# michael-fonder/M4Depth

Measured on AMD Instinct MI355X. Metric: frames/s, higher is better.
Workload: dtype f32

## Files before the change

include/m4depth_hip.h:

```cpp
#ifndef M4DEPTH_HIP_H_
#define M4DEPTH_HIP_H_

#include <stdint.h>

#ifdef __cplusplus
extern "C" {
#endif

#define M4D_ABI_VERSION 6

int m4d_abi_version(void);
long long m4d_launch_count(void);
const char* m4d_build_info(void);
const char* m4d_switches_info(void);


int m4d_backproject_fwd(const float* input, const float* coords, const int dims[6],
                        float* out, void* stream);

int m4d_backproject_bwd(const float* grad, const float* input, const float* coords,
                        const int dims[6], float* input_grad, float* coords_grad, void* stream);


int m4d_dense_image_warp(const float* image, const float* flow, int B, int H, int W, int C,
// ... 7 lines not shown
                       const float* cam_f, const float* cam_c, int b, int h, int w,
                       float* out, void* stream);
int m4d_depth2parallax(const float* depth, const float* rot, int rot_c, const float* trans,
                       const float* cam_f, const float* cam_c, int b, int h, int w,
                       float* out, void* stream);
int m4d_prev_d2para(const float* prev_d, const float* rot, int rot_c, const float* trans,
                    const float* cam_f, const float* cam_c, int b, int h, int w,
                    float* out, void* stream);
int m4d_reproject_flow(const float* depth, const float* rot, int rot_c, const float* trans,
                       const float* cam_f, const float* cam_c, int b, int h, int w,
                       float* flow, float* proj_minus_rot, float* rot_coord, void* stream);
int m4d_recompute_depth(const float* depth, const float* rot, int rot_c, const float* trans,
                        const float* cam_f, const float* cam_c, int b, int h, int w,
                        float* out, void* stream);


int m4d_dscv_fwd(const float* c1, const float* c2, const float* disp_prev_t, const float* disp,
                 const float* rot, int rot_c, const float* trans, const float* cam_f,
                 const float* cam_c, int b, int h, int w, int C, int search_range, int nbre_cuts,
                 int cv_accum, float* cv, int cv_stride, float* prev_disp,
                 float* log_center, int log_stride, float log_scale,
                 int32_t* index_out, void* stream);

void m4d_dscv_set_variant(int variant);
void m4d_dscv_set_fallback_counter(unsigned int* device_counter);
void m4d_dscv_set_ablation(int mask);
void m4d_dscv_set_stamps(unsigned long long* device_buffer);

int m4d_sncv_fwd(const float* c1, const float* c2, int b, int h, int w, int C, int search_range,
                 int dilation_rate, int nbre_cuts, float* out, int out_stride, void* stream);
int m4d_dscv_sncv_fwd(const float* c1, const float* c2, const float* disp_prev_t, const float* disp,
                      const float* rot, int rot_c, const float* trans, const float* cam_f,
                      const float* cam_c, int b, int h, int w, int C, int search_range, int nbre_cuts,
                      int cv_accum, float* cv, int cv_stride, float* prev_disp,
                      float* log_center, int log_stride, float log_scale,
                      int sncv_search_range, float* sncv_out, int sncv_out_stride, void* stream);

int m4d_conv3x3_wino_bias_act(const float* x, const float* wu, const float* bias, int b, int h, int w,
                              int Cin, int Cout, int CoutPad, float slope, float* out, void* stream);
int m4d_conv3x3_wino2_bias_act(const float* x, const float* wu8, const float* bias, int b, int h, int w,
                               int Cin, int Cout, int CoutPad, float slope, float* out, void* stream);
void m4d_wino_set_stamps(unsigned long long* device_buffer);
int m4d_conv3x3_wino6_bias_act(const float* x, const void* wu6, const float* bias, int b, int h, int w,
                               int Cin, int Cout, int CoutPad, float slope, float* out, void* stream);
int m4d_conv3x3_wino6_bias_act_k(const float* x, const void* wu6, const float* bias, int b, int h, int w,
                                 int Cin, int Cout, int CoutPad, float slope, float* out, int kernel, void* stream);
long long m4d_wino6_persistent_min_units(void);
void m4d_wino6_set_stamps(unsigned long long* device_buffer);
int m4d_conv3x3_wino6_bias_act_ks(const float* x, const void* wu6, const float* bias, int b, int h, int w,
                                  int Cin, int Cout, int CoutPad, float slope, float* out, int kernel,
                                  int stagger_us, int stagger_phases, void* stream);
int m4d_conv3x3_winof16_bias_act_ks(const float* x, const void* wuh, const float* bias, int b, int h, int w,
                                    int Cin, int Cout, int CoutPad, float slope, float* out,
                                    int stagger_us, int stagger_phases, void* stream);

int m4d_refiner_tail(const float* x32, const float* w6p, const float* b6, const float* w7p, const float* b7,
                     const float* rot, int rot_c, const float* trans, const float* cam_f, const float* cam_c,
                     int b, int h, int w, float scale, float* parallax, float* depth, float* other,
                     float* depth_state, void* stream);
int m4d_refiner_tail6(const float* x32, const void* w6f, const float* b6, const void* w7f, const float* b7,
                      const float* rot, int rot_c, const float* trans, const float* cam_f, const float* cam_c,
                      int b, int h, int w, float scale, float* parallax, float* depth, float* other,
                      float* depth_state, void* stream);

int m4d_refiner_tail6_m(const float* x32, const void* w6f, const float* b6, const void* w7f, const float* b7,
                        const float* rot, int rot_c, const float* trans, const float* cam_f, const float* cam_c,
                        int b, int h, int w, float scale, float* parallax, float* depth, float* other,
                        float* depth_state, const unsigned char* reset, float reset_parallax, void* stream);
int m4d_refiner_tail_m(const float* x32, const float* w6p, const float* b6, const float* w7p, const float* b7,
                       const float* rot, int rot_c, const float* trans, const float* cam_f, const float* cam_c,
                       int b, int h, int w, float scale, float* parallax, float* depth, float* other,
                       float* depth_state, const unsigned char* reset, float reset_parallax, void* stream);
int m4d_level_post_m(const float* refiner_out, const float* rot, int rot_c, const float* trans,
                     const float* cam_f, const float* cam_c, int b, int h, int w, float scale,
                     float* parallax, float* depth, float* other, float* depth_state,
                     const unsigned char* reset, float reset_parallax, void* stream);
int m4d_stream_prepare(const unsigned char* new_traj, int force_all, const float* rot, int rot_c, const float* trans,
                       int b, unsigned char* reset, float* rot_out, float* trans_out, void* stream);


int m4d_dscv_bwd(const float* c1, const float* c2, const float* disp_prev_t, const float* disp,
                 const float* rot, int rot_c, const float* trans, const float* cam_f,
                 const float* cam_c, int b, int h, int w, int C, int search_range, int nbre_cuts,
                 const float* g_cv, int g_cv_stride, const float* g_prev_disp,
                 float* g_c1, float* g_c2, float* g_disp, float* g_disp_prev_t, void* stream);

int m4d_sncv_bwd(const float* c1, const float* c2, const float* out, int out_stride,
                 const float* g, int g_stride, int b, int h, int w, int C, int search_range,
                 int dilation_rate, int nbre_cuts, float slope, float* g_c1, float* g_c2,
                 void* stream);


int m4d_resize_bilinear_v1_bwd(const float* g_out, int b, int ih, int iw, int c, int oh, int ow,
                               float mul, float* g_in, void* stream);
int m4d_level_post_bwd(const float* refiner_out, const float* g_parallax, const float* g_depth,
                       const float* g_other, const float* rot, int rot_c, const float* trans,
                       const float* cam_f, const float* cam_c, int b, int h, int w, float scale,
                       float* g_refiner_out, void* stream);
int m4d_normalize_cuts_bwd(const float* x, const float* g, int b, int h, int w, int C, int nbre_cuts,
                           float* g_x, void* stream);
long long m4d_bias_act_bwd_workspace_floats(long long rows, int C);
int m4d_bias_act_bwd(const float* g, const float* out, long long rows, int C, float slope,
                     float* g_pre, float* g_bias, float* workspace, void* stream);
int m4d_pack_conv_weights(const float* w_ohwi, int O, int I, int transpose, float* wp, void* stream);
int m4d_pack_conv_weights_lat(const float* w_ohwi, int O, int I, int transpose, void* wp, void* stream);
long long m4d_loss_workspace_floats(void);
// ... 235 lines not shown
```

m4depth_amd/csrc/m4d_wino_f16.hip:

```cpp
#include <cstdlib>
#include "m4d_common.h"
#include "../../include/m4depth_hip.h"

namespace {

typedef float f32x16 __attribute__((ext_vector_type(16)));
typedef _Float16 f16x8 __attribute__((ext_vector_type(8)));
typedef unsigned u32x4 __attribute__((ext_vector_type(4)));
typedef int i32x4 __attribute__((ext_vector_type(4)));

struct WinoF16Args {
  const float* x; const unsigned char* wu; const short* wexp; const float* bias; float* out;
  int b, h, w, Cin, Cout, CoutPad, n_chunks, tiles_x, tiles_y;
  float slope;
  int phases;
  int stagger;
};

constexpr int kT = 16, kH = kT + 2;
constexpr int kJ = 10;
constexpr int kPix = 5;
constexpr int kRow = 2 * kJ * kPix;
constexpr int kRawUsed = kH * kRow;
constexpr int kRawDma = 29;
constexpr int kRawK = 4;
constexpr int kRawSlots = kRawDma * 64;
constexpr int kFrag = 4 * 1024;
constexpr int kBRingBytes = 4 * kFrag;
constexpr int kBRingOff = 2 * kRawSlots * 16;
constexpr int kEpiBytes = (4 * 4 * 2 * 32 * 36 + 32) * 4;
constexpr int kPmOff = kEpiBytes;
constexpr int kTsOff = kPmOff + kH * kH * 4;
constexpr int kLdsBytes = kTsOff + 16 * 64 * 4;
static_assert(kBRingOff + 4 * kBRingBytes <= kEpiBytes, "the K loop's LDS lies inside the epilogue's");
static_assert(kLdsBytes <= 160 * 1024, "LDS budget of one CU");

__device__ __forceinline__ void split2_pair(float v0, float v1, float S, unsigned& hi, unsigned& lo) {
  asm("v_fma_mixlo_f16 %0, %1, %2, 0" : "=v"(hi) : "v"(v0), "v"(S));
  asm("v_fma_mixhi_f16 %0, %1, %2, 0" : "+v"(hi) : "v"(v1), "v"(S));
  asm("v_fma_mixlo_f16 %0, %1, %2, -%3 op_sel_hi:[0,0,1]" : "=v"(lo) : "v"(v0), "v"(S), "v"(hi));
  asm("v_fma_mixhi_f16 %0, %1, %2, -%3 op_sel:[0,0,1] op_sel_hi:[0,0,1]" : "+v"(lo) : "v"(v1), "v"(S), "v"(hi));
}

__device__ __forceinline__ float max3_abs(float m, float a, float b) {
  asm("v_max3_f32 %0, %0, |%1|, |%2|" : "+v"(m) : "v"(a), "v"(b));
  return m;
}

__global__ void __launch_bounds__(512) __attribute__((amdgpu_waves_per_eu(2, 2)))
conv3x3_winof16_kernel(const WinoF16Args a) {
  extern __shared__ __align__(16) float lds[];
  asm volatile("" : : "s"(a.x), "s"(a.wu), "s"(a.out), "s"(a.bias));
  if (a.stagger > 0 && blockIdx.y == 0 && blockIdx.x < 256) {
    const unsigned phase = (blockIdx.x >> 3) & (unsigned)(a.phases - 1);
    const unsigned long long t_end = wall_clock64() + (unsigned long long)(phase * (unsigned)a.stagger) / (unsigned)a.phases;
    for (int spin = 0; spin < 512 && wall_clock64() < t_end; ++spin) __builtin_amdgcn_s_sleep(16);
  }
  float4* raw = reinterpret_cast<float4*>(lds);
  unsigned* pm = reinterpret_cast<unsigned*>(reinterpret_cast<unsigned char*>(lds) + kPmOff);
  int* ts = reinterpret_cast<int*>(reinterpret_cast<unsigned char*>(lds) + kTsOff);
  const unsigned lds_base = (unsigned)(size_t)(__attribute__((address_space(3))) float*)lds;

  const int t = threadIdx.x, lane = t & 63;
  const int wv = __builtin_amdgcn_readfirstlane(t >> 6);
  const int pr = wv & 3, mt = wv >> 2;
// ... 59 lines not shown
        const int c = c0 + 2 * cc;
        const int s = src0 + qq + ((c & 1) * kJ + (c >> 1)) * kPix;
        const float4 da = rbuf[s + ra * kRow], db = rbuf[s + rb_ * kRow];
        tv[c][4 * qq + 0] = __builtin_fmaf(sgn, db.x, da.x);
        tv[c][4 * qq + 1] = __builtin_fmaf(sgn, db.y, da.y);
        tv[c][4 * qq + 2] = __builtin_fmaf(sgn, db.z, da.z);
        tv[c][4 * qq + 3] = __builtin_fmaf(sgn, db.w, da.w);
      }
  };
  float Sc[4];
  auto gen_pair = [&](int c, int e, u32x4 (&A)[2]) {
    float v[2];
#pragma unroll
    for (int h = 0; h < 2; ++h) {
      const int ch = 2 * e + h;
      v[h] = c == 0 ? tv[0][ch] - tv[2][ch] : c == 1 ? tv[1][ch] + tv[2][ch] : c == 2 ? tv[2][ch] - tv[1][ch] : tv[1][ch] - tv[3][ch];
    }
    unsigned p_hi, p_lo;
    split2_pair(v[0], v[1], Sc[c], p_hi, p_lo);
    A[0][e] = p_hi; A[1][e] = p_lo;
  };

  const long long w_pos = kFrag;
  const long long w_chunk = (long long)n_groups * 16 * w_pos;
  const unsigned char* wc = a.wu + ((long long)ng * 16 + 4 * pr) * w_pos;
  const unsigned bring = lds_base + (unsigned)(kBRingOff + pr * kBRingBytes);
  const unsigned char* bring_p = reinterpret_cast<const unsigned char*>(lds) + kBRingOff + pr * kBRingBytes;
  const unsigned bl = (unsigned)lane * 16u;
  const bool half = __builtin_amdgcn_readfirstlane(ng * 64 + 32 >= a.Cout ? 1 : 0) != 0;
  const unsigned bl_dma = (half && mt == 1) ? 0u : bl + (unsigned)mt * 2048u;
  auto b_dma = [&](const unsigned char* gsrc, int slot) {
    asm volatile("s_mov_b32 m0, %1\n\ts_nop 0\n\t"
                 "global_load_lds_dwordx4 %0, %2\n\tglobal_load_lds_dwordx4 %0, %2 offset:1024"
                 : : "v"(bl_dma), "s"(bring + (unsigned)(slot * kFrag) + (unsigned)mt * 2048u), "s"(gsrc) : "memory", "m0");
  };
  f16x8 B0[2][2], B1[2];
  auto frag = [&](int slot, int nt, int part) {
    return *reinterpret_cast<const f16x8*>(bring_p + slot * kFrag + (nt * 2 + part) * 1024 + bl);
  };
#define M4D_WF_WAIT(nn) asm volatile("s_waitcnt vmcnt(" #nn ") lgkmcnt(0)" ::: "memory")

  f32x16 acc[4][2];

#pragma unroll
  for (int k = 0; k < kRawK; ++k) raw_dma(0, 0, k);
  b_dma(wc, 0);
  b_dma(wc + w_pos, 1);
  b_dma(wc + 2 * w_pos, 2);
#pragma unroll
  for (int k = 0; k < kRawK; ++k) raw_dma(min(1, last), 1, k);
  b_dma(wc + 3 * w_pos, 3);
  static_assert(kRawK == 4, "the vmcnt counts below assume 4 raw-halo pieces + 2 fragment pieces per position");

  {
    const int g = t & 7, p0 = t >> 3, nq = a.Cin >> 2;
    constexpr int kR = (kH * kH + 63) / 64;
    int poff[kR];
    bool pv[kR];
    float mx[kR];
#pragma unroll
    for (int r = 0; r < kR; ++r) {
      const int p = p0 + 64 * r, hy = p / kH, hx = p - hy * kH;
      const int gy = tile_y - 1 + hy, gx = tile_x - 1 + hx;
      pv[r] = p < kH * kH && gy >= 0 && gy < a.h && gx >= 0 && gx < a.w;
      poff[r] = pv[r] ? (gy * a.w + gx) * a.Cin : 0;
      mx[r] = 0.f;
    }
#pragma unroll 2
    for (int q = g; q < nq; q += 8) {
#pragma unroll
      for (int r = 0; r < kR; ++r) {
        const float4 v = *reinterpret_cast<const float4*>(ximg + poff[r] + 4 * q);
        mx[r] = max3_abs(max3_abs(mx[r], v.x, v.y), v.z, v.w);
      }
    }
#pragma unroll
    for (int r = 0; r < kR; ++r) {
      unsigned u = pv[r] ? min(__float_as_uint(mx[r]), 0x7f7fffffu) : 0u;
      u = max(u, (unsigned)__builtin_amdgcn_update_dpp(0, (int)u, 0x141, 0xf, 0xf, false));
      u = max(u, (unsigned)__builtin_amdgcn_update_dpp(0, (int)u, 0xb1, 0xf, 0xf, false));
      u = max(u, (unsigned)__builtin_amdgcn_update_dpp(0, (int)u, 0x4e, 0xf, 0xf, false));
      const int p = p0 + 64 * r;
      if (g == 0 && p < kH * kH) pm[p] = u;
    }
  }
  __syncthreads();
  {
    const unsigned* row = pm + 2 * (4 * mt + ty0) * kH + 2 * tx;
    unsigned cm[4];
#pragma unroll
    for (int j = 0; j < 4; ++j) cm[j] = max(row[ra * kH + j], row[rb_ * kH + j]);
    const unsigned um[4] = {max(cm[0], cm[2]), max(cm[1], cm[2]), max(cm[1], cm[2]), max(cm[1], cm[3])};
#pragma unroll
    for (int c = 0; c < 4; ++c) {
      const int s = min(139 - (int)(um[c] >> 23), 126);
      Sc[c] = __uint_as_float((unsigned)(s + 127) << 23);
      if (kh == 0) ts[(pr * 4 + c) * 64 + mt * 32 + m] = -s;
    }
  }
  M4D_WF_WAIT(0);
  __syncthreads();
  u32x4 A[2][2];

  auto pin_a = [&](u32x4 (&X)[2]) {
#pragma unroll
    for (int part = 0; part < 2; ++part) asm volatile("" : "+v"(X[part]));
  };
// ... 123 lines not shown
#pragma unroll
        for (int r = 0; r < 16; ++r) {
          const int4 q = ne[c][r >> 2];
          const int ex = (r & 3) == 0 ? q.x : (r & 3) == 1 ? q.y : (r & 3) == 2 ? q.z : q.w;
          acc[c][nt][r] = __builtin_ldexpf(acc[c][nt][r], ex);
        }
    }
  }
#pragma unroll
  for (int nt = 0; nt < 2; ++nt) {
    if (nt == 1 && half) break;
    float* rbuf = Rb + (nt * 2 + mt) * kRbMT + nt * kRbSkew;
#pragma unroll
    for (int r = 0; r < 16; ++r) {
      const float m0 = acc[0][nt][r], m1 = acc[1][nt][r], m2 = acc[2][nt][r], m3 = acc[3][nt][r];
      const int trow = (r & 3) + 8 * (r >> 2) + 4 * kh;
      rbuf[((pr * 2 + 0) * 32 + trow) * kMS + m] = (m0 + m1) + m2;
      rbuf[((pr * 2 + 1) * 32 + trow) * kMS + m] = (m1 - m2) - m3;
    }
  }
  __syncthreads();
  float* oimg = a.out + (long long)bi * a.h * a.w * a.Cout;
  const bool vec_ok = (a.Cout & 3) == 0;
  const bool whole = tile_x + kT <= a.w && tile_y + kT <= a.h;
  const bool fast = whole && vec_ok && ng * 64 + (half ? 32 : 64) <= a.Cout;
  const int ont = cq16 >> 3, cq = cq16 & 7;
#pragma unroll
  for (int it = 0; it < 2; ++it) {
    if (it == 1 && half) break;
    const int tl = half ? (t >> 3) & 31 : (t >> 4) & 31, omt = half ? (t >> 8) : it;
    const float* rbuf = Rb + (ont * 2 + omt) * kRbMT + ont * kRbSkew;
    const int tg = omt * 32 + tl;
    const int ty2 = tg >> 3, tx2 = tg & 7;
    float4 rv[4][2];
#pragma unroll
    for (int i = 0; i < 4; ++i)
#pragma unroll
      for (int k = 0; k < 2; ++k) rv[i][k] = *reinterpret_cast<const float4*>(rbuf + ((i * 2 + k) * 32 + tl) * kMS + 4 * cq);
    float y[2][2][4];
#pragma unroll
    for (int k = 0; k < 2; ++k) {
      const float* r0 = reinterpret_cast<const float*>(&rv[0][k]); const float* r1 = reinterpret_cast<const float*>(&rv[1][k]);
      const float* r2 = reinterpret_cast<const float*>(&rv[2][k]); const float* r3 = reinterpret_cast<const float*>(&rv[3][k]);
#pragma unroll
      for (int e = 0; e < 4; ++e) {
        const int ex = -wt[e];
        const float v0 = __builtin_ldexpf((r0[e] + r1[e]) + r2[e], ex) + bs[e];
        const float v1 = __builtin_ldexpf((r1[e] - r2[e]) - r3[e], ex) + bs[e];
        y[k][0][e] = v0 > 0.f ? v0 : v0 * a.slope;
        y[k][1][e] = v1 > 0.f ? v1 : v1 * a.slope;
      }
    }
    const int ox = tile_x + 2 * tx2, oy = tile_y + 2 * ty2;
    float* op = oimg + ((long long)oy * a.w + ox) * a.Cout + co;
    if (fast) {
#pragma unroll
      for (int l = 0; l < 2; ++l)
#pragma unroll
        for (int k = 0; k < 2; ++k) m4d_store16(op + ((long long)l * a.w + k) * a.Cout, y[k][l][0], y[k][l][1], y[k][l][2], y[k][l][3]);
    } else if (co < a.Cout) {
#pragma unroll
      for (int l = 0; l < 2; ++l)
#pragma unroll
        for (int k = 0; k < 2; ++k)
          if (ox + k < a.w && oy + l < a.h) {
            float* o2 = op + ((long long)l * a.w + k) * a.Cout;
            if (vec_ok && co + 3 < a.Cout) m4d_store16(o2, y[k][l][0], y[k][l][1], y[k][l][2], y[k][l][3]);
            else { for (int e = 0; e < 4; ++e) if (co + e < a.Cout) o2[e] = y[k][l][e]; }
          }
    }
  }
}

}

extern "C" int m4d_conv3x3_winof16_bias_act_ks(const float* x, const void* wuh, const float* bias, int b, int h, int w,
                                               int Cin, int Cout, int CoutPad, float slope, float* out,
                                               int stagger_us, int stagger_phases, void* stream) {
  M4D_CHECK_ARG(x && wuh && bias && out && b > 0 && h > 0 && w > 0 && Cin >= 16 && Cout > 0);
  M4D_CHECK_ARG(CoutPad % 64 == 0 && CoutPad >= Cout && Cin % 16 == 0);
  M4D_CHECK_ARG(((((uintptr_t)x) & 15u) == 0) && ((((uintptr_t)wuh) & 15u) == 0));
  M4D_CHECK_ARG((long long)h * w * Cin * 4 < (1ll << 31));
  M4D_CHECK_ARG(stagger_us >= 0 && stagger_us <= 1000);
  M4D_CHECK_ARG(stagger_us == 0 || (stagger_phases >= 1 && stagger_phases <= 32 && !(stagger_phases & (stagger_phases - 1))));
  WinoF16Args a;
  a.x = x; a.wu = reinterpret_cast<const unsigned char*>(wuh); a.bias = bias; a.out = out;
  a.b = b; a.h = h; a.w = w; a.Cin = Cin; a.Cout = Cout; a.CoutPad = CoutPad; a.n_chunks = Cin / 16; a.slope = slope;
  a.wexp = reinterpret_cast<const short*>(a.wu + (long long)a.n_chunks * (CoutPad / 64) * 16 * kFrag);
  a.tiles_x = (w + kT - 1) / kT; a.tiles_y = (h + kT - 1) / kT;
  a.stagger = stagger_us * 100;
  a.phases = stagger_us > 0 ? stagger_phases : 1;
  const dim3 grid((unsigned)(a.tiles_x * a.tiles_y * (CoutPad / 64)), (unsigned)b);
  M4D_LDS_OPT_IN(&conv3x3_winof16_kernel);
  m4d_launch(conv3x3_winof16_kernel, grid, dim3(512), (size_t)kLdsBytes, (hipStream_t)stream, a);
  return M4D_LAUNCH_RESULT();
}
```

m4depth_amd/network.py:

```python
from __future__ import annotations

from collections import namedtuple

import numpy as np
import torch

from . import depth_operations as dops
from . import network_ops as nops
from ._lib import as_f32, lib
from .synthetic import ENCODER_CHANNELS, REFINER_CHANNELS, f_input_channels, nbre_cuts_for

M4depthAblationParameters = namedtuple('M4depthAblationParameters',
                                       ('DINL', 'SNCV', 'time_recurr', 'normalize_features',
                                        'subdivide_features', 'level_memory'),
                                       defaults=(True, True, True, True, True, True))

import contextlib as _contextlib
import os as _os

kernel_timer = None
debug_tap = None


winograd_conv = _os.environ.get("M4D_WINOGRAD", "1") == "1"
_WINO2_MIN_WORKGROUPS = 60

conv_arith = _os.environ.get("M4D_CONV_ARITH", "f16x2")
_SPLIT_ARITHS = ("bf16x3", "f16x2")
wino6_min_workgroups = int(_os.environ.get("M4D_WINO6_MIN_WG", "30"))
wino6_kernel = int(_os.environ.get("M4D_WINO6_KERNEL", "0"))
_WINO6_MIN_COUT = 32
small_conv_split = conv_arith in _SPLIT_ARITHS

tail_split = _os.environ.get("M4D_TAIL_SPLIT", "1") == "1"

encoder_batch_dispatch = _os.environ.get("M4D_ENCODER_BATCH_DISPATCH", "1") == "1"


@_contextlib.contextmanager
def conv_arithmetic(arith):
    global conv_arith, small_conv_split
    if arith not in _SPLIT_ARITHS + ("f32",):
        raise ValueError(f"conv arithmetic must be 'f16x2', 'bf16x3' or 'f32', not {arith!r}")
    old = (conv_arith, small_conv_split)
    conv_arith, small_conv_split = arith, arith in _SPLIT_ARITHS
    try:
        yield
    finally:
        conv_arith, small_conv_split = old


def _use_winograd(b, h, w, cin, cout, stride):
    if not winograd_conv or stride != 1 or cin < 16 or cin % 2 != 0:
        return 0
    n32 = -(-cout // 32)
    t16 = b * (-(-h // 16)) * (-(-w // 16))
    if conv_arith in _SPLIT_ARITHS and cin % 16 == 0 and cin >= 32 and cout >= _WINO6_MIN_COUT and t16 * (-(-cout // 64)) >= wino6_min_workgroups:
        return 6
    if cin % 4 == 0 and t16 * n32 >= _WINO2_MIN_WORKGROUPS:
        return 2
    t8 = b * (-(-h // 8)) * (-(-w // 16))
    if cout % 64 == 0 and t8 * (cout // 64) >= 400:
        return 1
    if cout >= 96 and 400 <= t8 * n32 <= 3000:
        return 1
    return 0


def _padded_refiner_width(f_in):
    return (f_in + 7) // 8 * 8


small_map_conv_pixels = int(_os.environ.get("M4D_CONV_SMALL_PX", "2048"))

lat_conv_max_pixels = int(_os.environ.get("M4D_LAT_CONV_PX", "2048"))

fused_front = _os.environ.get("M4D_FUSED_FRONT", "1") == "1"
fused_front_min_pixels = int(_os.environ.get("M4D_FUSED_FRONT_MIN_PX", "0"))
fused_front_coarse_min_pixels = int(_os.environ.get("M4D_FUSED_FRONT_COARSE_MIN_PX", "6000"))
_SMALL_CV_MAX_PIXELS = 6000

fused_refiner_tail = _os.environ.get("M4D_FUSED_TAIL", "1") == "1"

level_pipeline_streams = int(_os.environ.get("M4D_LEVEL_PIPELINE", "8"))
_PIPELINE_FORK_FRAMES = (1, 2)
wino6_stagger_us = int(_os.environ.get("M4D_WINO6_STAGGER_US", "9"))
_WINO6_STAGGER_PHASES = 16
_WINO6_STAGGER_MIN_WG = 200
_WINO6_STAGGER_MAX_BATCH = 4
wino6_stagger_autotune = _os.environ.get("M4D_STAGGER_AUTOTUNE", "1") == "1"
wino6_stagger_force = _os.environ.get("M4D_STAGGER_FORCE", "")
fused_pyramid_reset = _os.environ.get("M4D_FUSED_RESET", "1") == "1"
fused_encoder_level0 = _os.environ.get("M4D_FUSED_ENC0", "1") == "1"
pipeline_encoder_split = int(_os.environ.get("M4D_PIPELINE_ENCODER_SPLIT", "2"))
encoder_splitk_frames = 2
encoder_stats_up_front = _os.environ.get("M4D_ENC_STATS_UP_FRONT", "1") == "1"


def _stack_frames(samples):
    ims = [s['RGB_im'] for s in samples]
    x0 = ims[0]
    if (x0.is_cuda and x0.dtype == torch.float32 and x0.dim() == 4 and x0[0].is_contiguous()
            and all(x.dtype == x0.dtype and x.shape == x0.shape and x.stride() == x0.stride()
                    and x.untyped_storage().data_ptr() == x0.untyped_storage().data_ptr() for x in ims)):
        if len(ims) == 1:
            return nops.FrameStack(x0.unsqueeze(1))
        st = ims[1].storage_offset() - x0.storage_offset()
        if st > 0 and all(ims[t].storage_offset() - x0.storage_offset() == t * st for t in range(len(ims))):
            b, h, w, c = x0.shape
            return nops.FrameStack(torch.as_strided(x0, (b, len(ims), h, w, c), (x0.stride(0), st, w * c, c, 1),
                                                    x0.storage_offset()))
    return torch.cat([as_f32(x, "RGB_im") for x in ims], dim=0)


def _timed(name, level, thunk):
    kt = kernel_timer
    return thunk() if kt is None else kt.run(name, level, thunk)


def _to_device_f32(x, device):
    if isinstance(x, torch.Tensor):
        return x.to(device=device, dtype=torch.float32)
    return torch.as_tensor(np.asarray(x), dtype=torch.float32, device=device)


def _starts_trajectory(new_traj):
    if isinstance(new_traj, bool):
        return new_traj
# ... 93 lines not shown
            return cin == 3 or (self.stride == 2 and cin == 16 and cout == 16)
        if layout == "wino16":
            return wino
        if layout == "wino8":
            return wino and cin % 4 == 0
        if layout in ("wino6", "winof16"):
            return wino and cin % 16 == 0 and cin >= 32 and cout >= _WINO6_MIN_COUT
        if layout == "small6":
            return small and cin <= 256
        if layout in ("lat", "lat_f16"):
            return small
        raise KeyError(layout)

    def packed(self, layout, cin_pad=None):
        if layout == "hwio":
            return self._cache.get(("hwio",), _stamp(self.weight), lambda: self.weight.detach().permute(2, 3, 1, 0).contiguous())
        if cin_pad is not None and cin_pad == self.weight.shape[1]:
            cin_pad = None
        pack, int16, has_cout_pad = _LAYOUTS[layout]

        def build():
            assert self.can_use(layout, cin_pad or self.weight.shape[1]), (self.tag, layout, cin_pad)
            res = pack(self._hwio_numpy(cin_pad))
            wp, cpad = res if has_cout_pad else (res, None)
            wp = torch.from_numpy(wp.view("int16") if int16 else wp).to(self.weight.device)
            return (wp, cpad) if has_cout_pad else wp
        return self._cache.get((layout, cin_pad), _stamp(self.weight), build)

    def lat_f16(self):
        return conv_arith == "f16x2" and self.stride == 1

    def lat_eligible(self, b, h, w, cin):
        if not (self.small_maps_ok and conv_arith in _SPLIT_ARITHS and cin >= 16 and cin % 4 == 0 and self.stride == 1):
            return False
        eff_b = self.dispatch_batch if self.per_image_dispatch else b
        return eff_b * h * w <= lat_conv_max_pixels

    def splitk_batch(self):
        return self.dispatch_batch * encoder_splitk_frames if self.per_image_dispatch else None

    def same_pads(self, h, w):
        s = self.stride
        ph = max((-(-h // s) - 1) * s + 3 - h, 0)
        pw = max((-(-w // s) - 1) * s + 3 - w, 0)
        return (ph // 2, ph - ph // 2), (pw // 2, pw - pw // 2)

    def launch_stagger_us(self, b, h, w):
        us = wino6_stagger_us if self.wino6_stagger_us is None else self.wino6_stagger_us
        if us <= 0 or b > _WINO6_STAGGER_MAX_BATCH:
            return 0
        units = b * (-(-h // 16)) * (-(-w // 16)) * (-(-self.out_channels // 64))
        return int(us) if units >= _WINO6_STAGGER_MIN_WG else 0

    def plan(self, b, h, w, cin, final=True):
        eff_b = self.dispatch_batch if self.per_image_dispatch else b
        cout, s = self.out_channels, self.stride
        if self.lat_eligible(b, h, w, cin):
            kernel = "lat_f16" if self.lat_f16() else "lat"
            p = ConvPlan(kernel, kernel, nops.lat_config(eff_b, h, w, cin, cout, final), None, None)
            return p
        wino = _use_winograd(eff_b, h, w, cin, cout, s)
        one_launch = (not wino and self.small_maps_ok and 16 <= cin <= 256 and cin % 4 == 0
                      and eff_b * (-(-h // s)) * (-(-w // s)) <= small_map_conv_pixels)
        if wino == 6:
            p = ConvPlan("wino6", "winof16" if conv_arith == "f16x2" else "wino6", None, wino6_kernel,
                         self.launch_stagger_us(b, h, w))
        elif wino:
            p = ConvPlan("wino", "wino16", None, None, None) if wino == 1 else ConvPlan("wino2", "wino8", None, None, None)
        elif one_launch and s == 1 and small_conv_split:
            p = ConvPlan("small6", "small6", None, None, None)
        elif one_launch:
            p = ConvPlan("small", "direct", None, None, None)
        else:
            p = ConvPlan("direct", "direct", None, None, None)
        return p

    def forward(self, x_nhwc, slope=None, final=True):
        if isinstance(x_nhwc, nops.PartialAct) and not self.lat_eligible(*x_nhwc.shape):
            x_nhwc = x_nhwc.dense()
        if not x_nhwc.is_cuda:
            raise RuntimeError("m4depth_amd convolutions run on the GPU only (libm4depth_hip.so): got a CPU tensor; "
                               "there is no CPU fallback")
        if self.weight is None:
            self._build(x_nhwc.shape[-1], x_nhwc.device)
        if self.stride not in (1, 2):
            raise ValueError(f"stride {self.stride} is not supported by the HIP convolution")
        p = self.plan(*x_nhwc.shape, final)
        wts = self.packed(p.layout, x_nhwc.shape[-1])
        launch = _CONV_LAUNCH[p.kernel][1]
        act = 1.0 if slope is None else slope
        return _timed("conv", self.tag, lambda: launch(self, x_nhwc, wts, act, p))


ConvPlan = namedtuple("ConvPlan", ("kernel", "layout", "lat_config", "wino6_kernel", "stagger_us"))
LevelPlan = namedtuple("LevelPlan", ("route", "normalize", "f_stride", "tail"))

_LAYOUTS = {
    "direct": (nops.pack_conv_weights, False, True),
    "wino16": (lambda k: nops.pack_conv_weights_winograd(k, chunk=16), False, True),
    "wino8": (lambda k: nops.pack_conv_weights_winograd(k, chunk=8), False, True),
    "small6": (nops.pack_conv_weights_small6, True, True),
    "lat": (nops.pack_conv_weights_lat, True, False),
    "lat_f16": (nops.pack_conv_weights_lat_f16, True, False),
    "wino6": (nops.pack_conv_weights_wino6, True, True),
    "winof16": (nops.pack_conv_weights_winof16, True, True),
    "hwio": (None, False, False),
}

_CONV_LAUNCH = {
    "lat": ("conv3x3_lat", lambda c, x, w, act, p: nops.conv3x3_lat(
        x, w, c.bias, c.out_channels, act, config=p.lat_config, stride=c.stride)),
    "lat_f16": ("conv3x3_lat_f16", lambda c, x, w, act, p: nops.conv3x3_lat_f16(
        x, w, c.bias, c.out_channels, act, config=p.lat_config)),
    "wino6": ("conv3x3_wino6_bias_act", lambda c, x, w, act, p: nops.conv3x3_wino6_bias_act(
        x, w[0], c.bias, c.out_channels, w[1], act, kernel=p.wino6_kernel, stagger_us=p.stagger_us,
        stagger_phases=_WINO6_STAGGER_PHASES, arith=conv_arith)),
    "wino": ("conv3x3_wino_bias_act", lambda c, x, w, act, p: nops.conv3x3_wino_bias_act(
        x, w[0], c.bias, c.out_channels, w[1], act)),
    "wino2": ("conv3x3_wino2_bias_act", lambda c, x, w, act, p: nops.conv3x3_wino2_bias_act(
        x, w[0], c.bias, c.out_channels, w[1], act)),
    "small6": ("conv3x3_small6_bias_act", lambda c, x, w, act, p: nops.conv3x3_small6_bias_act(
        x, w[0], c.bias, c.out_channels, w[1], act)),
    "small": ("conv3x3_small_bias_act", lambda c, x, w, act, p: nops.conv3x3_small_bias_act(
        x, w[0], c.bias, c.out_channels, w[1], act, stride=c.stride)),
    "direct": ("conv3x3_bias_act", lambda c, x, w, act, p: nops.conv3x3_bias_act(
        x, w[0], c.bias, c.out_channels, w[1], act, stride=c.stride, split_batch=c.splitk_batch())),
}


class DomainNormalization(torch.nn.Module):

    def __init__(self, regularizer_weight=0.0004):
        super().__init__()
        self.regularizer_weight = regularizer_weight
        self.scale = None
        self.bias = None

    def _build(self, channels, device):
        self.scale = torch.nn.Parameter(torch.ones(1, 1, 1, channels, device=device), requires_grad=False)
        self.bias = torch.nn.Parameter(torch.zeros(1, 1, 1, channels, device=device), requires_grad=False)

    def forward(self, f_map, slope=1.0):
        if self.scale is None:
            self._build(f_map.shape[-1], f_map.device)
        if not f_map.is_cuda:
            raise RuntimeError("m4depth_amd DomainNormalization runs on the GPU only (libm4depth_hip.so): got a CPU tensor; "
                               "there is no CPU fallback")
        if f_map.shape[-1] not in (16, 32):
            raise ValueError(f"DomainNormalization: the HIP kernel is instantiated for 16 and 32 channels, not {f_map.shape[-1]}")
        return nops.dinl_act(f_map, self.scale, self.bias, slope)


class FeaturePyramid(torch.nn.Module):

    def __init__(self, settings, regularizer_weight=0.0004, trainable=True):
        super().__init__()
        self.use_dinl = settings["ablation"].DINL
        self.out_sizes = ENCODER_CHANNELS[:settings["nbre_lvls"]]
        cin = [3] + self.out_sizes[:-1]
        self.conv_layers_s1 = torch.nn.ModuleList([_Conv3x3SameTF(n, 1, ci) for n, ci in zip(self.out_sizes, cin)])
        self.conv_layers_s2 = torch.nn.ModuleList([_Conv3x3SameTF(n, 2, n) for n in self.out_sizes])
        self.dn_layers = torch.nn.ModuleList([DomainNormalization(regularizer_weight) for _ in self.out_sizes])
        for conv in list(self.conv_layers_s1) + list(self.conv_layers_s2):
            conv.per_image_dispatch = True
            conv.small_maps_ok = True

    def set_sequence_batch(self, b):
        b = max(int(b), 1) if encoder_batch_dispatch else 1
        for conv in list(self.conv_layers_s1) + list(self.conv_layers_s2):
# ... 213 lines not shown
            return {"depth": depth_prev_l, "parallax": para_prev_l, "other": other_prev_l}

        ab, k, lvl = self.ablation, self.nbre_cuts, self.lvl_depth
        scale = float(2.0 ** self.lvl_mul)
        f_input = nops.RefinerInput.for_level(lvl, b, h, w, self.f_in, p.f_stride, (2 * self.dscv_range + 1) * k,
                                              ab.level_memory, ab.time_recurr, dev)
        para_prev_l = para_prev_t = None
        if p.route in ("dscv_sncv", "dscv+sncv"):
            para_prev_l, _, _, para_prev_t = _timed("pre", lvl, lambda: nops.level_pre(
                prev_l_est, as_f32(prev_t_depth, "prev_t_depth"), trans, camera, b, h, w, dev, f_input=f_input, log_scale=scale,
                normalize=norm_job))
        rot_t = as_f32(rot, "rot")
        tr = as_f32(trans, "trans").reshape(b, 3)
        cf = as_f32(camera["f"], "camera['f']").reshape(b, 2)
        cc = as_f32(camera["c"], "camera['c']").reshape(b, 2)
        if rot_t.dim() != 2 or rot_t.shape[1] not in (3, 4):
            raise ValueError('Rotation must be expressed as a small angle (x,y,z) or a quaternion (w,x,y,z)')
        motion = (rot_t, tr, cf, cc)
        prev_f = as_f32(prev_f_maps, "prev_f_maps")
        cv = (k, self.dscv_range, self.sncv_range, self.cv_accum, f_input, scale)
        timed_as, opening = {
            "front": ("front", lambda: nops.level_front(
                curr_f_maps, curr_f, prev_f, as_f32(prev_t_depth, "prev_t_depth"), prev_l_est, motion, *cv)),
            "front_small": ("dscv_sncv", lambda: nops.level_front(
                None, curr_f, prev_f, as_f32(prev_t_depth, "prev_t_depth"), prev_l_est, motion, *cv)),
            "dscv_sncv": ("dscv_sncv", lambda: nops.dscv_sncv(curr_f, prev_f, para_prev_t, para_prev_l, motion, *cv)),
            "dscv+sncv": ("dscv", lambda: dops._dscv_forward(
                curr_f, prev_f, para_prev_t, para_prev_l, *motion, self.dscv_range, k, self.cv_accum, False,
                into=f_input.dscv_into(scale))),
        }[p.route]
        _timed(timed_as, lvl, opening)
        if p.route == "dscv+sncv" and ab.SNCV:
            _timed("sncv", lvl, lambda: dops._sncv_forward(curr_f, curr_f, self.sncv_range, 1, k, into=f_input.sncv_into()))
        self.last_f_input = f_input.rows()
        self.last_cv_inputs = (curr_f, prev_f, para_prev_t, para_prev_l, rot_t, tr, cf, cc)
        self.last_front_inputs = (curr_f_maps, prev_l_est, prev_t_depth)
        if debug_tap is not None:
            debug_tap("encoder_map", lvl, curr_f_maps)
            debug_tap("f_input", lvl, self.last_f_input)
        close_kw = {"depth_state": None if self.is_training else self.depth_prev_t}
        if reset_mask is not None:
            close_kw.update(reset=reset_mask, reset_parallax=float(reset_parallax))
        camera_t = {"f": cf, "c": cc}
        if p.tail == "post":
            prev_out = self.disp_refiner(f_input.buf)
            para_curr_l, depth, other = _timed("post", lvl, lambda: nops.level_post(
                prev_out[0], rot_t, tr, camera_t, scale, **close_kw))
        else:
            convs = list(self.disp_refiner.prep_conv_layers) + list(self.disp_refiner.est_d_conv_layers)
            x = f_input.buf
            for ci, conv in enumerate(convs[:5]):
                x = conv(x, slope=0.1, final=(ci == 4))
                if debug_tap is not None:
                    debug_tap(f"refiner_conv{ci + 1}", lvl, x.dense() if isinstance(x, nops.PartialAct) else x)
            w6p, w7p = self._tail_weights(convs, p.tail == "tail6")
            tail_fn = {"tail6": nops.refiner_tail6, "tail": nops.refiner_tail}[p.tail]
            para_curr_l, depth, other = _timed("tail", lvl, lambda: tail_fn(
                x, w6p, convs[5].bias, w7p, convs[6].bias, rot_t, tr, camera_t, scale, **close_kw))
        if not self.is_training:
            self.prev_f_maps = curr_f
        return {"other": other, "depth": depth, "parallax": para_curr_l}


def anti_diagonals(frames, n_lvls):
    frames = list(frames)
    return [(frames[i], diag - i) for diag in range(len(frames) + n_lvls - 1)
            for i in range(max(0, diag - n_lvls + 1), min(len(frames), diag + 1))]


class DepthEstimatorPyramid(torch.nn.Module):

    def __init__(self, settings, regularizer_weight=0.0004, trainable=True):
        super().__init__()
        self.levels = torch.nn.ModuleList(
            [DepthEstimatorLevel(settings, i + 1, regularizer_weight=regularizer_weight)
             for i in range(settings["nbre_lvls"])])
        self.is_training = settings["is_training"]
        self.is_unsupervised = False

    def prenormalize(self, pyr, bsz):
        if self.is_training or pyr is None or not isinstance(pyr[0], torch.Tensor) or not pyr[0].is_cuda:
            return None
        jobs = self._prenormalized_levels(pyr, bsz)
        if not jobs:
            return None
        outs = _timed("norm", "levels", lambda: nops.normalize_levels([(pyr[lvl], self.levels[lvl].nbre_cuts) for lvl in jobs]))
        res = [None] * len(pyr)
        for lvl, o in zip(jobs, outs):
            res[lvl] = o
        return res

    def _prenormalized_levels(self, pyr, bsz):
        return [lvl for lvl, t in enumerate(pyr[:len(self.levels)])
                if t.dim() == 4 and self.levels[lvl].wants_prenormalized(bsz, t.shape[1], t.shape[2], t.shape[3])]

    @staticmethod
    def _frame_slice(npyr, j, bsz):
        return None if npyr is None else [None if t is None else t[j * bsz:(j + 1) * bsz] for t in npyr]

    def pipeline_streams_for(self, traj_samples, dev):
        n_streams = level_pipeline_streams if (dev.type == "cuda" and not self.is_training and len(traj_samples) > 1
                                               and not (kernel_timer is not None and getattr(kernel_timer, "enabled", True))) else 0
        if n_streams < 2:
            return 0
        frames = len(traj_samples)
        if frames <= n_streams:
            return frames
# ... 719 lines not shown
```

m4depth_amd/network_ops.py:

```python
from __future__ import annotations

import ctypes

import torch

from ._lib import lib, dptr, stream_ptr, check, as_f32
from .depth_operations import _CV_ACCUM


def normalize_cuts(x, nbre_cuts, out=None):
    x = as_f32(x, "x")
    b, h, w, C = x.shape
    if C % nbre_cuts != 0:
        raise ValueError(f"nbre_cuts={nbre_cuts} does not divide the {C} feature channels")
    if out is None:
        out = torch.empty_like(x)
    check(lib.m4d_normalize_cuts(dptr(x, "x"), b, h, w, C, int(nbre_cuts), dptr(out, "out"), stream_ptr()),
          "m4d_normalize_cuts")
    return out


def resize_bilinear_v1(x, out_h, out_w, mul=1.0):
    x = as_f32(x, "x")
    b, ih, iw, c = x.shape
# ... 841 lines not shown
    while wgs(mt, kw) > lat_max_workgroups and mt < 4 and fits(mt * 2, kw):
        mt *= 2
    return mt, kw, s_out


def conv3x3_lat(x, wp, bias, cout, slope=0.1, final=False, config=None, stride=1):
    if isinstance(x, PartialAct):
        xs, s_in, x_bias, x_slope = x.slabs, x.slabs.shape[0], x.bias, x.slope
        b, h, w, cin = x.shape
        slab = b * h * w * cin
    else:
        xs = as_f32(x, "x")
        s_in, x_bias, x_slope = 1, None, 1.0
        b, h, w, cin = xs.shape
        slab = 0
    mt, kw, s_out = config if config is not None else lat_config(b, h, w, cin, cout, final, stride)
    act = 1.0 if slope is None else float(slope)
    oh, ow = -(-h // stride), -(-w // stride)
    out = torch.empty((s_out, b, oh, ow, cout), dtype=torch.float32, device=xs.device)
    check(lib.m4d_conv3x3s_lat(dptr(xs, "x"), s_in, slab, dptr(x_bias, "x_bias"), float(x_slope), dptr(wp, "wp", torch.int16),
                               dptr(bias, "bias"), b, h, w, cin, int(cout), int(stride), act, mt, kw, s_out, dptr(out),
                               b * oh * ow * int(cout), stream_ptr()), "m4d_conv3x3s_lat")
    return out[0] if s_out == 1 else PartialAct(out, bias, act)


def conv3x3_lat_f16(x, wp, bias, cout, slope=0.1, final=False, config=None):
    if isinstance(x, PartialAct):
        xs, s_in, x_bias, x_slope = x.slabs, x.slabs.shape[0], x.bias, x.slope
        b, h, w, cin = x.shape
        slab = b * h * w * cin
    else:
        xs = as_f32(x, "x")
        s_in, x_bias, x_slope = 1, None, 1.0
        b, h, w, cin = xs.shape
        slab = 0
    mt, kw, s_out = config if config is not None else lat_config(b, h, w, cin, cout, final)
    act = 1.0 if slope is None else float(slope)
    out = torch.empty((s_out, b, h, w, cout), dtype=torch.float32, device=xs.device)
    check(lib.m4d_conv3x3_lat_f16(dptr(xs, "x"), s_in, slab, dptr(x_bias, "x_bias"), float(x_slope), dptr(wp, "wp", torch.int16),
                                  dptr(bias, "bias"), b, h, w, cin, int(cout), act, mt, kw, s_out, dptr(out),
                                  b * h * w * int(cout), stream_ptr()), "m4d_conv3x3_lat_f16")
    return out[0] if s_out == 1 else PartialAct(out, bias, act)


def conv3x3_small6_bias_act(x, wp6, bias, cout, cout_pad, slope=0.1):
    x = as_f32(x, "x")
    b, h, w, cin = x.shape
    out = torch.empty((b, h, w, cout), dtype=torch.float32, device=x.device)
    check(lib.m4d_conv3x3_small6_bias_act(dptr(x, "x"), dptr(wp6, "wp6", torch.int16), dptr(bias, "bias"), b, h, w, cin, int(cout),
                                          int(cout_pad), float(slope), dptr(out), stream_ptr()), "m4d_conv3x3_small6_bias_act")
    return out


def conv3x3_winof16_bias_act(x, wuh, bias, cout, cout_pad, slope=0.1, stagger_us=0, stagger_phases=16):
    x = as_f32(x, "x")
    b, h, w, cin = x.shape
    out = torch.empty((b, h, w, cout), dtype=torch.float32, device=x.device)
    check(lib.m4d_conv3x3_winof16_bias_act_ks(dptr(x, "x"), dptr(wuh, "wuh", torch.int16), dptr(bias, "bias"), b, h, w, cin,
                                              int(cout), int(cout_pad), float(slope), dptr(out), int(stagger_us),
                                              int(stagger_phases), stream_ptr()),
          "m4d_conv3x3_winof16_bias_act_ks")
    return out


def conv3x3_wino6_bias_act(x, wu6, bias, cout, cout_pad, slope=0.1, kernel=0, stagger_us=0, stagger_phases=16, arith="bf16x3"):
    if arith == "f16x2":
        return conv3x3_winof16_bias_act(x, wu6, bias, cout, cout_pad, slope, stagger_us=stagger_us, stagger_phases=stagger_phases)
    x = as_f32(x, "x")
    b, h, w, cin = x.shape
    out = torch.empty((b, h, w, cout), dtype=torch.float32, device=x.device)
    check(lib.m4d_conv3x3_wino6_bias_act_ks(dptr(x, "x"), dptr(wu6, "wu6", torch.int16), dptr(bias, "bias"), b, h, w, cin,
                                            int(cout), int(cout_pad), float(slope), dptr(out), int(kernel), int(stagger_us),
                                            int(stagger_phases), stream_ptr()),
          "m4d_conv3x3_wino6_bias_act_ks")
    return out


class FrameStack:

    def __init__(self, frames):
        if frames.dim() != 5 or frames.dtype != torch.float32 or not frames[0, 0].is_contiguous():
            raise ValueError("FrameStack: expected a float32 [b,T,H,W,3] view with dense frames")
        self.frames = frames

    @property
    def shape(self):
        bsz, t, h, w, c = self.frames.shape
        return (bsz * t, h, w, c)

    @property
    def is_cuda(self):
        return self.frames.is_cuda

    @property
    def device(self):
        return self.frames.device

    def dense(self):
        bsz, t, h, w, c = self.frames.shape
        return self.frames.transpose(0, 1).reshape(bsz * t, h, w, c)


def encoder_head(images, w_hwio, bias1, dn_scale, dn_bias, wp2, bias2, cout2, cout2_pad, slope=0.1):
    if isinstance(images, FrameStack):
        fr = images.frames
        bsz = fr.shape[0]
        stride_b, stride_t = fr.stride(0), fr.stride(1)
        b, h, w, c3 = images.shape
        img_ptr = ctypes.c_void_p(fr.data_ptr())
        if not fr.is_cuda:
            raise RuntimeError("images: m4depth_amd ops run on the MI355X only; there is no CPU fallback")
        images_dev = fr.device
    else:
        images = as_f32(images, "images")
        b, h, w, c3 = images.shape
        bsz, stride_b, stride_t = b, h * w * c3, 0
        img_ptr = dptr(images, "images")
        images_dev = images.device
    if c3 != 3:
        raise ValueError(f"encoder_head expects RGB images, got {c3} channels")
# ... 348 lines not shown
```

Before: 1821.

## Hand per-pixel activation maxima from one f16 Winograd conv to the next

The f16x2 Winograd conv epilogue can now also write per-pixel, per-64-channel-group absolute maxima of its output, reduced across lanes with DPP. The next f16 Winograd conv reads these maxima instead of rescanning its whole input halo to find per-pixel scale exponents. This removes a full input read pass per conv in chained refiner convs, at the cost of extra epilogue work, an extra small buffer write, and new plumbing (an ActMaxima wrapper) in the Python dispatch.

New measurement: 1855 (median of 6 runs). 1.9% higher.

```diff
diff --git a/include/m4depth_hip.h b/include/m4depth_hip.h
--- a/include/m4depth_hip.h
+++ b/include/m4depth_hip.h
@@ -83,6 +83,10 @@
                                   int stagger_us, int stagger_phases, void* stream);
 int m4d_conv3x3_winof16_bias_act_ks(const float* x, const void* wuh, const float* bias, int b, int h, int w,
                                     int Cin, int Cout, int CoutPad, float slope, float* out,
+                                    int stagger_us, int stagger_phases, void* stream);
+int m4d_conv3x3_winof16_bias_act_pm(const float* x, const void* wuh, const float* bias, int b, int h, int w,
+                                    int Cin, int Cout, int CoutPad, float slope, float* out,
+                                    const unsigned* pm_in, unsigned* pm_out,
                                     int stagger_us, int stagger_phases, void* stream);
 
 int m4d_refiner_tail(const float* x32, const float* w6p, const float* b6, const float* w7p, const float* b7,
diff --git a/m4depth_amd/csrc/m4d_wino_f16.hip b/m4depth_amd/csrc/m4d_wino_f16.hip
--- a/m4depth_amd/csrc/m4d_wino_f16.hip
+++ b/m4depth_amd/csrc/m4d_wino_f16.hip
@@ -11,6 +11,8 @@
 
 struct WinoF16Args {
   const float* x; const unsigned char* wu; const short* wexp; const float* bias; float* out;
+  const unsigned* pm_in;
+  unsigned* pm_out;
   int b, h, w, Cin, Cout, CoutPad, n_chunks, tiles_x, tiles_y;
   float slope;
   int phases;
@@ -176,7 +178,19 @@
   b_dma(wc + 3 * w_pos, 3);
   static_assert(kRawK == 4, "the vmcnt counts below assume 4 raw-halo pieces + 2 fragment pieces per position");
 
-  {
+  if (a.pm_in) {
+    if (t < kH * kH) {
+      const int hy = t / kH, hx = t - hy * kH;
+      const int gy = tile_y - 1 + hy, gx = tile_x - 1 + hx;
+      const int G = (a.Cin + 63) >> 6;
+      unsigned u = 0u;
+      if (gy >= 0 && gy < a.h && gx >= 0 && gx < a.w) {
+        const unsigned* q = a.pm_in + (((long long)bi * a.h + gy) * a.w + gx) * G;
+        for (int g = 0; g < G; ++g) u = max(u, q[g]);
+      }
+      pm[t] = min(u, 0x7f7fffffu);
+    }
+  } else {
     const int g = t & 7, p0 = t >> 3, nq = a.Cin >> 2;
     constexpr int kR = (kH * kH + 63) / 64;
     int poff[kR];
@@ -406,6 +420,35 @@
       }
     }
     const int ox = tile_x + 2 * tx2, oy = tile_y + 2 * ty2;
+    if (a.pm_out) {
+      const bool allv = ng * 64 + (half ? 32 : 64) <= a.Cout;
+      unsigned pu[2][2];
+#pragma unroll
+      for (int k = 0; k < 2; ++k)
+#pragma unroll
+        for (int l = 0; l < 2; ++l) {
+          float v[4];
+#pragma unroll
+          for (int e = 0; e < 4; ++e) v[e] = (allv || co + e < a.Cout) ? y[k][l][e] : 0.f;
+          pu[k][l] = min(__float_as_uint(max3_abs(max3_abs(0.f, v[0], v[1]), v[2], v[3])), 0x7f7fffffu);
+        }
+#define M4D_WF_PMAX(ctrl)                                                                                              \
+  _Pragma("unroll") for (int k = 0; k < 2; ++k) _Pragma("unroll") for (int l = 0; l < 2; ++l)                            \
+    pu[k][l] = max(pu[k][l], (unsigned)__builtin_amdgcn_update_dpp(0, (int)pu[k][l], ctrl, 0xf, 0xf, false));
+      M4D_WF_PMAX(0x141)
+      M4D_WF_PMAX(0xb1)
+      M4D_WF_PMAX(0x4e)
+      if (!half) { M4D_WF_PMAX(0x140) }
+#undef M4D_WF_PMAX
+      if (cq16 == 0) {
+        unsigned* pp = a.pm_out + (((long long)bi * a.h + oy) * a.w + ox) * n_groups + ng;
+#pragma unroll
+        for (int l = 0; l < 2; ++l)
+#pragma unroll
+          for (int k = 0; k < 2; ++k)
+            if (ox + k < a.w && oy + l < a.h) pp[((long long)l * a.w + k) * n_groups] = pu[k][l];
+      }
+    }
     float* op = oimg + ((long long)oy * a.w + ox) * a.Cout + co;
     if (fast) {
 #pragma unroll
@@ -428,8 +471,9 @@
 
 }
 
-extern "C" int m4d_conv3x3_winof16_bias_act_ks(const float* x, const void* wuh, const float* bias, int b, int h, int w,
+extern "C" int m4d_conv3x3_winof16_bias_act_pm(const float* x, const void* wuh, const float* bias, int b, int h, int w,
                                                int Cin, int Cout, int CoutPad, float slope, float* out,
+                                               const unsigned* pm_in, unsigned* pm_out,
                                                int stagger_us, int stagger_phases, void* stream) {
   M4D_CHECK_ARG(x && wuh && bias && out && b > 0 && h > 0 && w > 0 && Cin >= 16 && Cout > 0);
   M4D_CHECK_ARG(CoutPad % 64 == 0 && CoutPad >= Cout && Cin % 16 == 0);
@@ -437,7 +481,10 @@
   M4D_CHECK_ARG((long long)h * w * Cin * 4 < (1ll << 31));
   M4D_CHECK_ARG(stagger_us >= 0 && stagger_us <= 1000);
   M4D_CHECK_ARG(stagger_us == 0 || (stagger_phases >= 1 && stagger_phases <= 32 && !(stagger_phases & (stagger_phases - 1))));
+  M4D_CHECK_ARG(((((uintptr_t)pm_in) & 3u) == 0) && ((((uintptr_t)pm_out) & 3u) == 0));
+  M4D_CHECK_ARG(!pm_out || (CoutPad - Cout < 64 && (const void*)pm_out != (const void*)pm_in));
   WinoF16Args a;
+  a.pm_in = pm_in; a.pm_out = pm_out;
   a.x = x; a.wu = reinterpret_cast<const unsigned char*>(wuh); a.bias = bias; a.out = out;
   a.b = b; a.h = h; a.w = w; a.Cin = Cin; a.Cout = Cout; a.CoutPad = CoutPad; a.n_chunks = Cin / 16; a.slope = slope;
   a.wexp = reinterpret_cast<const short*>(a.wu + (long long)a.n_chunks * (CoutPad / 64) * 16 * kFrag);
@@ -449,3 +496,10 @@
   m4d_launch(conv3x3_winof16_kernel, grid, dim3(512), (size_t)kLdsBytes, (hipStream_t)stream, a);
   return M4D_LAUNCH_RESULT();
 }
+
+extern "C" int m4d_conv3x3_winof16_bias_act_ks(const float* x, const void* wuh, const float* bias, int b, int h, int w,
+                                               int Cin, int Cout, int CoutPad, float slope, float* out,
+                                               int stagger_us, int stagger_phases, void* stream) {
+  return m4d_conv3x3_winof16_bias_act_pm(x, wuh, bias, b, h, w, Cin, Cout, CoutPad, slope, out, nullptr, nullptr, stagger_us,
+                                         stagger_phases, stream);
+}
diff --git a/m4depth_amd/network.py b/m4depth_amd/network.py
--- a/m4depth_amd/network.py
+++ b/m4depth_amd/network.py
@@ -74,6 +74,9 @@
 small_map_conv_pixels = int(_os.environ.get("M4D_CONV_SMALL_PX", "2048"))
 
 lat_conv_max_pixels = int(_os.environ.get("M4D_LAT_CONV_PX", "2048"))
+
+wino_handover = _os.environ.get("M4D_WINO_HANDOVER", "1") == "1"
+_WINO_HANDOVER_MIN_TILES = 100
 
 fused_front = _os.environ.get("M4D_FUSED_FRONT", "1") == "1"
 fused_front_min_pixels = int(_os.environ.get("M4D_FUSED_FRONT_MIN_PX", "0"))
@@ -273,7 +276,7 @@
         units = b * (-(-h // 16)) * (-(-w // 16)) * (-(-self.out_channels // 64))
         return int(us) if units >= _WINO6_STAGGER_MIN_WG else 0
 
-    def plan(self, b, h, w, cin, final=True):
+    def plan(self, b, h, w, cin, final=True, maxima=False):
         eff_b = self.dispatch_batch if self.per_image_dispatch else b
         cout, s = self.out_channels, self.stride
         if self.lat_eligible(b, h, w, cin):
@@ -284,8 +287,11 @@
         one_launch = (not wino and self.small_maps_ok and 16 <= cin <= 256 and cin % 4 == 0
                       and eff_b * (-(-h // s)) * (-(-w // s)) <= small_map_conv_pixels)
         if wino == 6:
-            p = ConvPlan("wino6", "winof16" if conv_arith == "f16x2" else "wino6", None, wino6_kernel,
-                         self.launch_stagger_us(b, h, w))
+            hand = (conv_arith == "f16x2" and wino_handover
+                    and b * (-(-h // 16)) * (-(-w // 16)) >= _WINO_HANDOVER_MIN_TILES)
+            p = ConvPlan("wino6", "winof16" if conv_arith == "f16x2" else "wino6", None, wino6_kernel, self.launch_stagger_us(b, h, w),
+                         bool(hand and maxima and self.weight is not None and cin == self.weight.shape[1]),
+                         bool(hand and not final))
         elif wino:
             p = ConvPlan("wino", "wino16", None, None, None) if wino == 1 else ConvPlan("wino2", "wino8", None, None, None)
         elif one_launch and s == 1 and small_conv_split:
@@ -299,6 +305,7 @@
     def forward(self, x_nhwc, slope=None, final=True):
         if isinstance(x_nhwc, nops.PartialAct) and not self.lat_eligible(*x_nhwc.shape):
             x_nhwc = x_nhwc.dense()
+        maxima = isinstance(x_nhwc, nops.ActMaxima)
         if not x_nhwc.is_cuda:
             raise RuntimeError("m4depth_amd convolutions run on the GPU only (libm4depth_hip.so): got a CPU tensor; "
                                "there is no CPU fallback")
@@ -306,14 +313,17 @@
             self._build(x_nhwc.shape[-1], x_nhwc.device)
         if self.stride not in (1, 2):
             raise ValueError(f"stride {self.stride} is not supported by the HIP convolution")
-        p = self.plan(*x_nhwc.shape, final)
+        p = self.plan(*x_nhwc.shape, final, maxima)
+        if maxima and not p.reads_maxima:
+            x_nhwc = x_nhwc.dense()
         wts = self.packed(p.layout, x_nhwc.shape[-1])
         launch = _CONV_LAUNCH[p.kernel][1]
         act = 1.0 if slope is None else slope
         return _timed("conv", self.tag, lambda: launch(self, x_nhwc, wts, act, p))
 
 
-ConvPlan = namedtuple("ConvPlan", ("kernel", "layout", "lat_config", "wino6_kernel", "stagger_us"))
+ConvPlan = namedtuple("ConvPlan", ("kernel", "layout", "lat_config", "wino6_kernel", "stagger_us", "reads_maxima", "writes_maxima"),
+                      defaults=(False, False))
 LevelPlan = namedtuple("LevelPlan", ("route", "normalize", "f_stride", "tail"))
 
 _LAYOUTS = {
@@ -335,7 +345,7 @@
         x, w, c.bias, c.out_channels, act, config=p.lat_config)),
     "wino6": ("conv3x3_wino6_bias_act", lambda c, x, w, act, p: nops.conv3x3_wino6_bias_act(
         x, w[0], c.bias, c.out_channels, w[1], act, kernel=p.wino6_kernel, stagger_us=p.stagger_us,
-        stagger_phases=_WINO6_STAGGER_PHASES, arith=conv_arith)),
+        stagger_phases=_WINO6_STAGGER_PHASES, arith=conv_arith, want_maxima=p.writes_maxima)),
     "wino": ("conv3x3_wino_bias_act", lambda c, x, w, act, p: nops.conv3x3_wino_bias_act(
         x, w[0], c.bias, c.out_channels, w[1], act)),
     "wino2": ("conv3x3_wino2_bias_act", lambda c, x, w, act, p: nops.conv3x3_wino2_bias_act(
@@ -655,7 +665,7 @@
             for ci, conv in enumerate(convs[:5]):
                 x = conv(x, slope=0.1, final=(ci == 4))
                 if debug_tap is not None:
-                    debug_tap(f"refiner_conv{ci + 1}", lvl, x.dense() if isinstance(x, nops.PartialAct) else x)
+                    debug_tap(f"refiner_conv{ci + 1}", lvl, x.dense() if isinstance(x, (nops.PartialAct, nops.ActMaxima)) else x)
             w6p, w7p = self._tail_weights(convs, p.tail == "tail6")
             tail_fn = {"tail6": nops.refiner_tail6, "tail": nops.refiner_tail}[p.tail]
             para_curr_l, depth, other = _timed("tail", lvl, lambda: tail_fn(
diff --git a/m4depth_amd/network_ops.py b/m4depth_amd/network_ops.py
--- a/m4depth_amd/network_ops.py
+++ b/m4depth_amd/network_ops.py
@@ -917,20 +917,57 @@
     return out
 
 
-def conv3x3_winof16_bias_act(x, wuh, bias, cout, cout_pad, slope=0.1, stagger_us=0, stagger_phases=16):
+class ActMaxima:
+
+    def __init__(self, tensor, maxima):
+        self.tensor, self.maxima = tensor, maxima
+
+    @property
+    def shape(self):
+        return self.tensor.shape
+
+    @property
+    def is_cuda(self):
+        return self.tensor.is_cuda
+
+    @property
+    def device(self):
+        return self.tensor.device
+
+    def dense(self):
+        return self.tensor
+
+
+def conv3x3_winof16_bias_act(x, wuh, bias, cout, cout_pad, slope=0.1, stagger_us=0, stagger_phases=16, want_maxima=False):
+    pm_in = None
+    if isinstance(x, ActMaxima):
+        x, pm_in = x.tensor, x.maxima
     x = as_f32(x, "x")
     b, h, w, cin = x.shape
     out = torch.empty((b, h, w, cout), dtype=torch.float32, device=x.device)
-    check(lib.m4d_conv3x3_winof16_bias_act_ks(dptr(x, "x"), dptr(wuh, "wuh", torch.int16), dptr(bias, "bias"), b, h, w, cin,
-                                              int(cout), int(cout_pad), float(slope), dptr(out), int(stagger_us),
-                                              int(stagger_phases), stream_ptr()),
-          "m4d_conv3x3_winof16_bias_act_ks")
-    return out
-
-
-def conv3x3_wino6_bias_act(x, wu6, bias, cout, cout_pad, slope=0.1, kernel=0, stagger_us=0, stagger_phases=16, arith="bf16x3"):
+    if pm_in is None and not want_maxima:
+        check(lib.m4d_conv3x3_winof16_bias_act_ks(dptr(x, "x"), dptr(wuh, "wuh", torch.int16), dptr(bias, "bias"), b, h, w, cin,
+                                                  int(cout), int(cout_pad), float(slope), dptr(out), int(stagger_us),
+                                                  int(stagger_phases), stream_ptr()),
+              "m4d_conv3x3_winof16_bias_act_ks")
+        return out
+    if pm_in is not None and tuple(pm_in.shape) != (b, h, w, -(-cin // 64)):
+        raise ValueError(f"conv3x3_winof16_bias_act: maxima {tuple(pm_in.shape)} do not belong to an input {tuple(x.shape)}")
+    pm_out = torch.empty((b, h, w, int(cout_pad) // 64), dtype=torch.int32, device=x.device) if want_maxima else None
+    check(lib.m4d_conv3x3_winof16_bias_act_pm(dptr(x, "x"), dptr(wuh, "wuh", torch.int16), dptr(bias, "bias"), b, h, w, cin,
+                                              int(cout), int(cout_pad), float(slope), dptr(out), dptr(pm_in, "maxima", torch.int32),
+                                              dptr(pm_out, "maxima", torch.int32), int(stagger_us), int(stagger_phases), stream_ptr()),
+          "m4d_conv3x3_winof16_bias_act_pm")
+    return ActMaxima(out, pm_out) if want_maxima else out
+
+
+def conv3x3_wino6_bias_act(x, wu6, bias, cout, cout_pad, slope=0.1, kernel=0, stagger_us=0, stagger_phases=16, arith="bf16x3",
+                           want_maxima=False):
     if arith == "f16x2":
-        return conv3x3_winof16_bias_act(x, wu6, bias, cout, cout_pad, slope, stagger_us=stagger_us, stagger_phases=stagger_phases)
+        return conv3x3_winof16_bias_act(x, wu6, bias, cout, cout_pad, slope, stagger_us=stagger_us, stagger_phases=stagger_phases,
+                                        want_maxima=want_maxima)
+    if want_maxima or isinstance(x, ActMaxima):
+        raise ValueError("conv3x3_wino6_bias_act: pixel maxima are handed on by the f16x2 kernel only")
     x = as_f32(x, "x")
     b, h, w, cin = x.shape
     out = torch.empty((b, h, w, cout), dtype=torch.float32, device=x.device)
```
